# databendlabs/databend

Hardware: AMD Instinct MI355X
Metric: rows/s TPC-H Q1 hash-agg (higher is better)
Workload: dtype i64/i128 decimal

## Files before the change

### databend_amd/csrc/fagg_device.h

```cpp
#pragma once
#include "dev_expr.h"
#include "gb_device.h"

namespace {

constexpr int FA_MAX_SLOTS = 8;
constexpr int FA_KW = 4;
constexpr int FA_MAXW = 12;
constexpr int FA_MAXA = 8;
#ifndef DBHIP_JIT
constexpr int FA_ROWS = 2;
#endif

enum { W_NONE = 0, W_ADD1, W_ADD3, W_FADD, W_OR, W_MIN, W_MAX, W_CONT };
enum { C_LO = 0, C_HI, C_EXT, C_FLAG, C_ENC };

struct FaKeyTable {
  uint32_t count;
  uint32_t lock;
  uint64_t key[FA_MAX_SLOTS][FA_KW];
};
typedef volatile __attribute__((address_space(3))) FaKeyTable* FaKeyTableV;
#define FA_LDS_V(T) ((FaKeyTableV)(T))

// ... 270 lines not shown
      carry = (uint64_t)cout;
    }
  }
}
template <bool GENERAL, int NW>
__device__ __forceinline__ void fa_wave_fold(uint64_t (&v)[NW], const uint32_t (&wm)[NW]) {
#pragma nounroll
  for (int off = 32; off >= 1; off >>= 1) {
    uint64_t o[NW];
#pragma unroll
    for (int w = 0; w < NW; ++w) o[w] = __shfl_xor(v[w], off, 64);
    fa_fold_words<GENERAL, NW>(v, o, wm);
  }
}

template <int SLOTS, bool GENERAL, int NW, bool DIV = false>
__device__ __forceinline__ void fagg_body(const FaArgs& A) {
  extern __shared__ uint64_t ex_lds[];
  __shared__ FaKeyTable T;
  __shared__ uint32_t wm_lds[FA_MAXW];
  __shared__ uint32_t wg_touched;
  __shared__ unsigned long long wg_row0;
  __shared__ uint64_t fa_xw[4][SLOTS][NW];
#ifdef DBHIP_JIT
  const FaArgs& M = kM;
  uint64_t ex_rf[EX_MAX_SLOTS * FA_ROWS];
  uint64_t* const ex_regs = ex_rf;
#define EX_REG(r, k) ex_regs[(r) * FA_ROWS + (k)]
#else
  const FaArgs& M = A;
  uint64_t* const ex_regs = ex_lds;
#define EX_REG(r, k) ex_regs[((r) * FA_ROWS + (k)) * 256 + tid]
#endif
  const ExProg& P = M.P;
  const ExProg& PA = A.P;
  const int tid = threadIdx.x, lane = tid & 63;
  if (tid == 0) { T.count = 0; T.lock = 0; wg_touched = 0; }
  if (tid < FA_MAX_SLOTS * FA_KW) T.key[tid / FA_KW][tid % FA_KW] = 0;
  if (tid < FA_MAXW) wm_lds[tid] = M.wm[tid];
  __syncthreads();

  uint32_t wm[NW];
#pragma unroll
  for (int w = 0; w < NW; ++w) {
#ifdef DBHIP_JIT
    wm[w] = M.wm[w];
#else
    wm[w] = __builtin_amdgcn_readfirstlane(A.wm[w]);
#endif
  }
  uint64_t acc[SLOTS][NW];
  uint32_t touched = 0;
// ... 198 lines not shown
              }
            } else if (GENERAL && op == W_CONT && WM_COMP(m) == C_FLAG) {
            } else {
              const unsigned long long cin = WM_CARRY(m) ? (unsigned long long)carry : 0ULL;
              unsigned long long cout;
              acc[g][w] = (uint64_t)__builtin_addcll((unsigned long long)acc[g][w], (unsigned long long)val[w], cin, &cout);
              carry = (uint64_t)cout;
            }
          }
        }
      }
    }
  }
  flags = (uint32_t)fa_wave_or((uint64_t)flags);
  if (lane == 0 && flags) atomicOr((unsigned long long*)&A.ctrl[1], (unsigned long long)flags);
  const uint32_t wt = (uint32_t)fa_wave_or((uint64_t)touched);
  if (lane == 0 && wt) atomicOr(&wg_touched, wt);
  const int wave = tid >> 6;
#pragma unroll
  for (int g = 0; g < SLOTS; ++g) {
    if ((wt >> g) & 1) fa_wave_fold<GENERAL, NW>(acc[g], wm);
    if (lane == 0) {
#pragma unroll
      for (int w = 0; w < NW; ++w) fa_xw[wave][g][w] = acc[g][w];
    }
  }
  __syncthreads();
  const uint32_t tw = wg_touched;
  if (tw == 0) return;
  if (tid == 0) wg_row0 = atomicAdd((unsigned long long*)&A.ctrl[0], (unsigned long long)__popc(tw));
  __syncthreads();
  if (tid < SLOTS && ((tw >> tid) & 1)) {
    const int g = tid;
    uint64_t v[NW];
#pragma unroll
    for (int w = 0; w < NW; ++w) v[w] = fa_xw[0][g][w];
#pragma unroll
    for (int x = 1; x < 4; ++x) {
      uint64_t o[NW];
#pragma unroll
      for (int w = 0; w < NW; ++w) o[w] = fa_xw[x][g][w];
      fa_fold_words<GENERAL, NW>(v, o, wm);
    }
    uint64_t* r = A.partial_rows + (wg_row0 + (unsigned long long)__popc(tw & ((1u << g) - 1u))) * M.W;
    uint64_t kk[FA_KW];
#pragma unroll
    for (int j = 0; j < FA_KW; ++j) kk[j] = T.key[g][j];
    uint64_t vmk = ~0ULL;
#pragma unroll
    for (int j = 0; j < FA_KW; ++j)
      if (j == M.validity_word) vmk = kk[j];
    uint64_t h = 0;
    for (int q = 0; q < M.nkeys; ++q) {
      uint64_t w2[2] = {0, 0};
#pragma unroll
      for (int j = 0; j < FA_KW; ++j) {
        if (j == M.key_off[q]) w2[0] = kk[j];
        if (M.key_words[q] == 2 && j == M.key_off[q] + 1) w2[1] = kk[j];
      }
      const uint64_t hk = gb_hash_words(M.key_type[q], w2, (vmk >> q) & 1);
      h = q == 0 ? hk : merge_hash(h, hk);
    }
#pragma unroll
    for (int j = 0; j < FA_KW; ++j)
      if (j < M.nkey_words) r[j] = kk[j];
    r[M.hash_word] = h;
    uint64_t* st = r + M.state_off;
#pragma unroll
    for (int w = 0; w < NW; ++w) {
      if (w >= M.nwords) continue;
      const uint32_t op = WM_OP(wm[w]);
      if (op == W_NONE) continue;
      const bool flag = op == W_OR || (GENERAL && op == W_CONT && WM_COMP(wm[w]) == C_FLAG);
      st[w] = flag ? (v[w] ? 1 : 0) : v[w];
    }
  }
#undef EX_REG
#undef FA_IN_DATA
#undef FA_IN_VALID
#undef FA_IN_VOFF
#undef FA_KEY_DATA
#undef FA_KEY_VALID
#undef FA_KEY_VOFF
#undef FA_FILTER_BITS
#undef FA_FILTER_OFF
}

#ifndef DBHIP_JIT
template <int SLOTS, bool GENERAL, int NW, bool DIV = false>
__global__ __launch_bounds__(256, (SLOTS * NW <= 16) ? 2 : 1) void fagg_kernel(FaArgs A) {
  fagg_body<SLOTS, GENERAL, NW, DIV>(A);
}
#endif

}
```

### databend_amd/csrc/gbk_merge_lds.h

```cpp

namespace {

int32_t ensure(void** p, size_t* cap, size_t bytes) {
  if (*cap >= bytes) return DBHIP_OK;
  if (*p) {
    int32_t rc = dbhip_free(*p);
    if (rc) return rc;
    *p = nullptr; *cap = 0;
  }
  size_t want = bytes + (bytes >> 3) + 256;
  int32_t rc = dbhip_alloc(want, p);
  if (rc) { *p = nullptr; return rc; }
  *cap = want;
  return DBHIP_OK;
}

int32_t alloc_table(dbhip_groupby* g, int64_t cap, hipStream_t s) {
  uint64_t* nh = nullptr;
  uint64_t* nr = nullptr;
  int32_t rc = dbhip_alloc((size_t)cap * 8, (void**)&nh);
  if (rc == DBHIP_OK) rc = dbhip_alloc((size_t)cap * g->L.W * 8, (void**)&nr);
  hipError_t e = rc == DBHIP_OK ? hipMemsetAsync(nh, 0, (size_t)cap * 8, s) : hipSuccess;
  if (rc != DBHIP_OK || e != hipSuccess) {
    if (nh) (void)dbhip_free(nh);
// ... 140 lines not shown
  g->arena_cap = want;
  return DBHIP_OK;
}
int32_t reserve_arena_for_chunk(dbhip_groupby* g, hipStream_t s) {
  uint64_t lb = 0;
  DBHIP_CHECK(hipMemcpyAsync(&lb, &g->ctrl[9], 8, hipMemcpyDeviceToHost, s));
  DBHIP_CHECK(hipStreamSynchronize(s));
  if (lb == 0) return DBHIP_OK;
  g->has_long = 1;
  return reserve_arena(g, lb, s);
}
bool layout_has_strings(const GbLayout& L) { return L.str_w1_mask != 0; }
bool layout_has_wide_minmax(const GbLayout& L);

int32_t merge_rows_unpinned(dbhip_groupby* g, const uint64_t* rows_in, int64_t n, hipStream_t s, const uint64_t* n_dev, const uint64_t* abort_dev,
                            int deferred = 0);
int32_t merge_rows(dbhip_groupby* g, const uint64_t* rows_in, int64_t n, hipStream_t s,
                   const uint64_t* n_dev = nullptr, const uint64_t* abort_dev = nullptr) {
  int32_t rc = merge_rows_unpinned(g, rows_in, n, s, n_dev, abort_dev);
  if (rc == DBHIP_OK && n > 0) rc = pin_string_states(g, s);
  return rc;
}
int32_t merge_rows_unpinned(dbhip_groupby* g, const uint64_t* rows_in, int64_t n, hipStream_t s,
                            const uint64_t* n_dev, const uint64_t* abort_dev, int deferred) {
  if (n == 0) return DBHIP_OK;
  if (n > 0xFFFFFFF0LL) {
    set_error("groupby: more than 2^32 rows in one call");
    return DBHIP_ERR_INVALID;
  }
  int32_t rc;
  if ((rc = ensure((void**)&g->gid, &g->gid_cap, (size_t)n * 4))) return rc;
  if ((rc = ensure((void**)&g->retry, &g->retry_cap, (size_t)n * 4))) return rc;
  const int grid = grid_for(n, 256);
  uint64_t* host_ctrl = pinned_words(0);
  if (!host_ctrl) return DBHIP_ERR_HIP;
  const uint64_t* cur_rows = rows_in;
  int64_t cur_n = n;
  const DevCount dc{n_dev, abort_dev};
  if ((deferred || (g->count_host + n) * 135 <= g->cap * 100) && n <= 256) {
    hipLaunchKernelGGL(gb_merge_small_kernel, dim3(1), dim3(256), 0, s, g->L, cur_rows, cur_n, g->slot_hash, g->rows, g->cap, g->hash_mask, g->gid,
                       g->retry, g->ctrl, dc, g->arena);
    DBHIP_LAUNCH_CHECK();
    if (deferred) return DBHIP_OK;
    DBHIP_CHECK(hipMemcpyAsync(host_ctrl, g->ctrl, 5 * sizeof(uint64_t), hipMemcpyDeviceToHost, s));
    DBHIP_CHECK(hipStreamSynchronize(s));
    g->count_host = (int64_t)host_ctrl[0];
    if (host_ctrl[3] & 2) {
      set_error("groupby: a string key longer than 12 bytes was met; keep the CPU operator for this block");
      return DBHIP_ERR_UNSUPPORTED;
    }
    if (host_ctrl[1]) {
      set_error("groupby: collision chain filled the table during retry; create the table with a larger capacity");
      return DBHIP_ERR_CAPACITY;
    }
    return DBHIP_OK;
  }
  if (deferred || (g->count_host + n) * 135 <= g->cap * 100) {
    DBHIP_CHECK(hipMemsetAsync(&g->ctrl[1], 0, 16, s));
    hipLaunchKernelGGL(gb_probe_kernel, dim3(grid), dim3(256), 0, s, g->L, cur_rows, cur_n, g->slot_hash, g->rows, g->cap,
                       g->hash_mask, g->gid, g->ctrl, dc, g->arena);
    if (deferred == 1 || (!deferred && g->count_host > 0 && g->count_host <= 32 && n <= 65536) || n <= 2048 || layout_has_wide_minmax(g->L))
      hipLaunchKernelGGL(gb_accum_lowcard_kernel, dim3(deferred == 1 && grid > 16 ? 16 : grid), dim3(256), 0, s, g->L, cur_rows, cur_n, g->rows, g->gid, g->retry,
                         g->ctrl, dc, g->arena);
    else
      hipLaunchKernelGGL(gb_accum_kernel, dim3(grid), dim3(256), 0, s, g->L, cur_rows, cur_n, g->rows, g->gid, g->retry, g->ctrl, dc, g->arena);
    hipLaunchKernelGGL(gb_retry_kernel, dim3(1), dim3(64), 0, s, g->L, cur_rows, g->slot_hash, g->rows, g->cap, g->hash_mask,
                       g->gid, g->retry, g->ctrl, g->arena);
    DBHIP_LAUNCH_CHECK();
    if (deferred) return DBHIP_OK;
    DBHIP_CHECK(hipMemcpyAsync(host_ctrl, g->ctrl, 5 * sizeof(uint64_t), hipMemcpyDeviceToHost, s));
// ... 315 lines not shown
```

### databend_amd/csrc/gbk_rows.h

```cpp

namespace {

struct HashCols {
  GbCol c[GB_MAX_KEYS];
  int n;
};

__global__ __launch_bounds__(256) void group_hash_kernel(HashCols hc, int64_t n, uint64_t* out,
                                                         unsigned long long* bad) {
  constexpr int U = 4;
  const int64_t T = (int64_t)gridDim.x * blockDim.x;
  const int64_t t = (int64_t)blockIdx.x * blockDim.x + threadIdx.x;
  for (int64_t base = 0; base < n; base += U * T) {
    int64_t row[U];
    bool in[U];
    uint64_t h[U];
#pragma unroll
    for (int u = 0; u < U; ++u) {
      row[u] = base + u * T + t;
      in[u] = row[u] < n;
      if (!in[u]) row[u] = n - 1;
      h[u] = 0;
    }
    for (int k = 0; k < hc.n; ++k) {
// ... 452 lines not shown
      }
      pos = (pos + 1) & cmask;
    }
    if (!done) ctrl[1] |= 2;
  }
}
__global__ void gb_retry_kernel(GbLayout L, const uint64_t* rows_in, uint64_t* slot_hash, uint64_t* rows,
                                int64_t cap, uint64_t hash_mask, const uint32_t* gid,
                                const uint32_t* retry, uint64_t* ctrl, uint8_t* arena) {
  if (threadIdx.x != 0 || blockIdx.x != 0) return;
  gb_retry_body(L, rows_in, slot_hash, rows, cap, hash_mask, gid, retry, ctrl, arena);
}

__global__ __launch_bounds__(256) void gb_merge_small_kernel(GbLayout L, const uint64_t* rows_in, int64_t n, uint64_t* slot_hash, uint64_t* rows,
                                                             int64_t cap, uint64_t hash_mask, uint32_t* gid, uint32_t* retry, uint64_t* ctrl,
                                                             DevCount dc, uint8_t* arena) {
  n = dev_rows(dc, n);
  if (threadIdx.x < 2) ctrl[1 + threadIdx.x] = 0;
  __threadfence();
  __syncthreads();
  gb_probe_body(L, rows_in, n, slot_hash, rows, cap, hash_mask, gid, ctrl, arena);
  __threadfence();
  __syncthreads();
  gb_accum_lowcard_body(L, rows_in, n, rows, gid, retry, ctrl, arena);
  __threadfence();
  __syncthreads();
  if (threadIdx.x == 0) gb_retry_body(L, rows_in, slot_hash, rows, cap, hash_mask, gid, retry, ctrl, arena);
}

__global__ __launch_bounds__(256) void gb_rehash_kernel(GbLayout L, const uint64_t* old_hash,
                                                        const uint64_t* old_rows, int64_t old_cap,
                                                        uint64_t* new_hash, uint64_t* new_rows,
                                                        int64_t new_cap, uint64_t hash_mask) {
  const uint64_t cmask = (uint64_t)new_cap - 1;
  for (int64_t s = (int64_t)blockIdx.x * blockDim.x + threadIdx.x; s < old_cap;
       s += (int64_t)gridDim.x * blockDim.x) {
    uint64_t hw = old_hash[s];
    if (hw == 0) continue;
    const uint64_t* r = old_rows + s * L.W;
    uint64_t pos = home_slot(probe_word(r[L.hash_word], hash_mask), new_cap);
    while (true) {
      unsigned long long old = atomicCAS((unsigned long long*)&new_hash[pos], 0ULL, (unsigned long long)hw);
// ... 501 lines not shown
```

### databend_amd/csrc/k_fagg.hip

```cpp
#include "fagg_device.h"
#include "runtime.h"

#include <dirent.h>
#include <dlfcn.h>
#include <errno.h>
#include <sys/stat.h>
#include <fcntl.h>
#include <signal.h>
#include <spawn.h>
#include <sys/wait.h>
#include <unistd.h>

#include <atomic>
#include <chrono>
#include <deque>
#include <map>
#include <mutex>
#include <string>

#include <stdlib.h>
#include <string.h>
#include <time.h>

using namespace dbhip;

int32_t dbhip_groupby_merge_rows_dev_internal(dbhip_groupby* g, const uint64_t* rows, int64_t n_max, const uint64_t* n_dev,
                                              const uint64_t* abort_dev, hipStream_t s);
int32_t dbhip_groupby_merge_rows_internal(dbhip_groupby* g, const uint64_t* rows, int64_t n, hipStream_t s);
int64_t dbhip_groupby_capacity_internal(dbhip_groupby* g);
int32_t dbhip_groupby_reserve_merge_internal(dbhip_groupby* g, int64_t n);
int64_t dbhip_groupby_count_internal(dbhip_groupby* g);
const GbLayout* dbhip_groupby_layout_internal(dbhip_groupby* g);
int32_t dbhip_groupby_merge_rows_deferred_internal(dbhip_groupby* g, const uint64_t* rows, int64_t n_max, const uint64_t* n_dev,
                                                   const uint64_t* abort_dev, hipStream_t s);
int32_t dbhip_groupby_ensure_room_internal(dbhip_groupby* g, int64_t extra, hipStream_t s);
uint64_t* dbhip_groupby_ctrl_internal(dbhip_groupby* g);
void dbhip_groupby_set_count_internal(dbhip_groupby* g, int64_t count);
void** dbhip_groupby_pipe_slot_internal(dbhip_groupby* g);

namespace {

#include "build/jit_embed.inc"

struct JitOut {
  std::string s;
  void num(long long v) { s += std::to_string(v); s += ","; }
  void u64(uint64_t v) { char b[40]; snprintf(b, sizeof(b), "0x%llxULL,", (unsigned long long)v); s += b; }
  void null() { s += "nullptr,"; }
  void open() { s += "{"; }
  void close() { s += "},"; }
};

void jit_ins(JitOut& o, const ExIns& I) {
// ... 271 lines not shown
  return ok;
}

struct JitEntry {
  enum State { ABSENT = 0, PENDING, READY, FAILED } state = ABSENT;
  hipModule_t mod = nullptr;
  hipFunction_t fn = nullptr;
  std::chrono::steady_clock::time_point checked{}, started{};
};
std::mutex g_jit_mu;
std::map<std::string, JitEntry> g_jit_cache;

int jit_mode() {
  static const int m = [] {
    const char* e = getenv("DBHIP_FAGG_JIT");
    if (!e) return 1;
    if (!strcmp(e, "sync")) return 2;
    return atoi(e) == 0 ? 0 : 1;
  }();
  return m;
}

enum { JIT_LOOKUP = 0, JIT_COMPILE = 1, JIT_BACKGROUND = 2 };
void fa_shape(const FaArgs& A, FaArgs& K) {
  K = A;
  for (int i = 0; i < EX_MAX_INPUTS; ++i) { K.P.in_data[i] = nullptr; K.P.in_valid[i] = nullptr; K.P.in_voff[i] = 0; }
  K.P.err_words = nullptr; K.P.err_count = nullptr;
  for (int k = 0; k < FA_KW; ++k) { K.key[k].data = nullptr; K.key[k].validity = nullptr; K.key[k].voff = 0; K.key[k].buffers = nullptr; }
  K.filter_bits = nullptr; K.filter_off = 0; K.n = 0; K.partial_rows = nullptr; K.ctrl = nullptr; K.blocks = nullptr; K.wgs_per_block = 0;
}
hipFunction_t jit_kernel(const FaArgs& A, int slots, bool general, int nw, int how, bool* pending = nullptr, bool multi = false) {
  if (pending) *pending = false;
  const int mode = jit_mode();
  if (mode == 0) return nullptr;
  if (mode == 2) how = JIT_COMPILE;
// ... 78 lines not shown
  return words <= FA_MAXW && L.hash_word == L.nkey_words && L.agg_off[0] == L.hash_word + 1;
}

static std::atomic<uint64_t> g_fa_jit_launches{0}, g_fa_interp_launches{0}, g_fa_pending_refusals{0}, g_fa_multi_blocks{0};
extern "C" int32_t dbhip_fagg_stats(uint64_t* out3_host) {
  DBHIP_REQUIRE(out3_host, "dbhip_fagg_stats: NULL argument");
  out3_host[0] = g_fa_jit_launches.load(); out3_host[1] = g_fa_interp_launches.load(); out3_host[2] = g_fa_pending_refusals.load();
  return DBHIP_OK;
}

static thread_local bool t_prepare_only = false;
static thread_local bool t_jit_only = false;
static thread_local bool t_jit_pending = false;
static thread_local bool t_jit_may_compile = true;

static int32_t fa_build_args(const GbLayout& L, const dbhip_col* keys, const dbhip_agg_program* prog, FaArgs& A, bool* out_general,
                             int* out_nwords, bool* out_may_raise) {
  ExRoot roots[EX_MAX_ROOTS + 1];
  int n_roots = 0, filter_root = -1;
  int root_of_agg[FA_MAXA];
  if (prog->filter_reg >= 0) { roots[n_roots].reg = prog->filter_reg; filter_root = n_roots++; }
  for (int a = 0; a < L.naggs; ++a) {
    root_of_agg[a] = -1;
    const int32_t r = prog->arg_regs[a];
    if (r == DBHIP_ARG_NONE) {
      if (L.agg_kind[a] != DBHIP_AGG_COUNT) { set_error("dbhip_groupby_add_block_program: aggregate %d needs an argument", a); return DBHIP_ERR_INVALID; }
      continue;
    }
    if (n_roots >= EX_MAX_ROOTS) { set_error("dbhip_groupby_add_block_program: more than %d program results", EX_MAX_ROOTS); return DBHIP_ERR_UNSUPPORTED; }
    roots[n_roots].reg = r;
// ... 1 lines not shown
  }
  bool may_raise = false, any_nullable = false;
  if (n_roots == 0) {
    set_error("dbhip_groupby_add_block_program: nothing to evaluate (count(*) only): use dbhip_groupby_add_block_filtered");
    return DBHIP_ERR_UNSUPPORTED;
  }
  int32_t rc = dbhip_expr_compile_internal(prog->prog, prog->n_ins, prog->inputs, prog->n_inputs, roots, n_roots, filter_root, &A.P,
                                           &may_raise, &any_nullable);
  if (rc) return rc;
  A.naggs = L.naggs;
  int nwords = 0;
  bool general = false;
  for (int a = 0; a < L.naggs; ++a) {
    int slot = 0, wide = 0, sgn = 0, enc_type = L.agg_type[a];
    uint32_t dep = 0;
    const int fw = L.agg_flag[a];
    const int base_words = L.agg_words[a] - (fw ? 1 : 0);
    if (root_of_agg[a] >= 0) {
      const ExRoot& R = roots[root_of_agg[a]];
      if (L.agg_kind[a] != DBHIP_AGG_COUNT) {
        if (R.type != L.agg_type[a] || !fa_arg_type_ok(R.type)) {
          set_error("dbhip_groupby_add_block_program: aggregate %d expects an argument of type %d, the program yields type %d", a, L.agg_type[a], R.type);
          return DBHIP_ERR_INVALID;
        }
      }
      slot = R.slot; wide = R.wide; dep = R.dep;
      sgn = R.type == DBHIP_T_DEC128 || type_class(R.type) == CLS_SIGNED;
      if (R.type == DBHIP_T_F32) enc_type = DBHIP_T_F64;
    }
    auto put = [&](int op, int comp, int carry_in) {
      A.wm[nwords++] = (uint32_t)op | ((uint32_t)comp << 3) | ((uint32_t)slot << 6) | ((uint32_t)wide << 12) | ((uint32_t)sgn << 13) |
                       ((uint32_t)carry_in << 14) | (1u << 15) | ((dep & 255u) << 16) | (((uint32_t)enc_type & 31u) << 24);
    };
    switch (L.agg_kind[a]) {
      case DBHIP_AGG_COUNT: put(W_ADD1, C_FLAG, 0); break;
      case DBHIP_AGG_SUM:
        if (base_words == 3) { put(W_ADD3, C_LO, 0); put(W_CONT, C_HI, 1); put(W_CONT, C_EXT, 1); }
        else if (L.agg_type[a] == DBHIP_T_F32 || L.agg_type[a] == DBHIP_T_F64) { put(W_FADD, C_LO, 0); general = true; }
        else put(W_ADD1, C_LO, 0);
        if (fw) put(W_OR, C_FLAG, 0);
        break;
      case DBHIP_AGG_MIN: case DBHIP_AGG_MAX:
        if (L.agg_words[a] >= 3) { set_error("fused aggregation: min / max over Decimal128 / Decimal256 / String stays on the row path"); return DBHIP_ERR_UNSUPPORTED; }
        if (L.agg_kind[a] == DBHIP_AGG_MIN) put(W_MIN, C_ENC, 0); else put(W_MAX, C_ENC, 0);
        put(W_CONT, C_FLAG, 0); general = true; break;
    }
  }
  A.nwords = nwords;
  A.state_off = L.agg_off[0];
  A.nkeys = L.nkeys; A.nkey_words = L.nkey_words; A.validity_word = L.validity_word; A.hash_word = L.hash_word; A.W = L.W;
  for (int k = 0; k < L.nkeys; ++k) {
    if (keys[k].type != L.key_type[k]) { set_error("dbhip_groupby_add_block_program: key %d has type %d, table expects %d", k, keys[k].type, L.key_type[k]); return DBHIP_ERR_INVALID; }
    if (keys[k].validity && !L.key_nullable[k]) { set_error("dbhip_groupby_add_block_program: key %d carries validity but was declared NOT NULL", k); return DBHIP_ERR_INVALID; }
    GbCol& c = A.key[k];
    c.data = keys[k].data; c.validity = keys[k].validity; c.voff = keys[k].validity_offset; c.buffers = keys[k].buffers;
    c.type = keys[k].type; c.is_scalar = keys[k].is_scalar;
    A.key_type[k] = L.key_type[k]; A.key_off[k] = L.key_off[k]; A.key_words[k] = L.key_words[k];
    A.key_has_valid[k] = keys[k].validity != nullptr;
  }
  *out_general = general; *out_nwords = nwords; *out_may_raise = may_raise;
  return DBHIP_OK;
// ... 20 lines not shown
#define FA_LAUNCH(SL, GEN)                                                                                     \
  do {                                                                                                         \
    if (nwords <= 4) hipLaunchKernelGGL((fagg_kernel<SL, GEN, 4>), dim3(grid), dim3(256), lds, s, A);           \
    else hipLaunchKernelGGL((fagg_kernel<SL, GEN, FA_MAXW>), dim3(grid), dim3(256), lds, s, A);                 \
  } while (0)
  bool has_div = false;
  for (int i = 0; i < A.P.n_ins; ++i) has_div |= A.P.ins[i].op == EX_DEC && dec_op_needs_division(A.P.dec[A.P.ins[i].dec_idx]);
  if (has_div && slots == 4) hipLaunchKernelGGL((fagg_kernel<4, true, FA_MAXW, true>), dim3(grid), dim3(256), lds, s, A);
  else if (has_div) hipLaunchKernelGGL((fagg_kernel<8, true, FA_MAXW, true>), dim3(grid), dim3(256), lds, s, A);
  else if (slots == 4 && !general) FA_LAUNCH(4, false);
  else if (slots == 4) FA_LAUNCH(4, true);
  else if (!general) FA_LAUNCH(8, false);
  else FA_LAUNCH(8, true);
#undef FA_LAUNCH
  return DBHIP_OK;
}

namespace {
constexpr int FA_PIPE_WINDOW = 2048;
constexpr int FA_PIPE_BATCH = 512;
constexpr size_t FA_PIPE_COPY_BYTES = 16384;
constexpr size_t FA_PIPE_TABLE_BYTES = 65536;
constexpr int FA_PIPE_RING = 8;
constexpr int64_t FA_PIPE_BIG = 8 << 20;
constexpr int64_t FA_PIPE_BATCH_ROWS = 32 << 20;
struct FaShape { FaArgs A; bool general; int nwords; size_t lds; std::string sig; };
struct FaPending { int shape; FaBlock b; };
struct FaMerge { uint64_t seq; int64_t rows_ub; int64_t blocks; };
struct FaPipe {
  bool on = false, bound = false, slots8 = false;
// ... 358 lines not shown
  int32_t rc = fa_build_args(L, keys, prog, A, &general, &nwords, &may_raise);
  if (rc) return rc;
  A.filter_bits = filter_bitmap; A.filter_off = filter_bit_offset; A.n = n;
  A.has_filter = filter_bitmap != nullptr;
  const size_t lds = (size_t)(A.P.n_slots > 6 ? A.P.n_slots : 6) * FA_ROWS * 256 * 8;
  if (lds > 60 * 1024) {
    set_error("dbhip_groupby_add_block_program: %d live LDS slots exceed the register file; split the expression", A.P.n_slots);
    return DBHIP_ERR_UNSUPPORTED;
  }
  const int64_t nchunks = ceil_div(n, 64 * FA_ROWS);
  const int grid = (int)(ceil_div(nchunks, 4) < 512 ? ceil_div(nchunks, 4) : 512);
  if (FaPipe* pp = (FaPipe*)*dbhip_groupby_pipe_slot_internal(g); pp && !t_prepare_only) {
    int64_t committed = 0;
    if ((rc = fa_pipe_checkpoint(g, pp, &committed, true))) return rc;
  }
  const size_t rows_bytes = (size_t)grid * FA_MAX_SLOTS * L.W * 8;
  uint8_t* ws = (uint8_t*)scratch(rows_bytes + 64, 6, s);
  if (!ws) return DBHIP_ERR_HIP;
  uint64_t* ctrl = (uint64_t*)ws;
  A.ctrl = ctrl;
  A.partial_rows = (uint64_t*)(ws + 64);
  A.P.err_words = nullptr;
  A.P.err_count = (unsigned long long*)&ctrl[2];
  uint64_t* host_ctrl = pinned_words(1);
  if (!host_ctrl) return DBHIP_ERR_HIP;
  host_ctrl[0] = host_ctrl[1] = host_ctrl[2] = 0;
  const int64_t n_max = (int64_t)grid * FA_MAX_SLOTS;
  const bool chained = (dbhip_groupby_count_internal(g) + n_max) * 135 <= dbhip_groupby_capacity_internal(g) * 100;
  if ((rc = dbhip_groupby_reserve_merge_internal(g, n_max))) return rc;
  if (t_prepare_only) {
    (void)jit_kernel(A, dbhip_groupby_count_internal(g) > 4 ? 8 : 4, general, nwords, JIT_COMPILE);
    if (FaPipe* pq = (FaPipe*)*dbhip_groupby_pipe_slot_internal(g); pq && pq->on)
      (void)jit_kernel(A, dbhip_groupby_count_internal(g) > 4 ? 8 : 4, general, nwords, JIT_COMPILE, nullptr, true);
    return DBHIP_OK;
  }
  for (int variant = dbhip_groupby_count_internal(g) > 4 ? 1 : 0; variant < 2; ++variant) {
    DBHIP_CHECK(hipMemsetAsync(ctrl, 0, 64, s));
    kernel_timer_start(s);
    if ((rc = fa_launch(A, variant == 0 ? 4 : 8, general, nwords, grid, lds, s))) return rc;
    kernel_timer_stop(s);
    DBHIP_LAUNCH_CHECK();
    DBHIP_CHECK(hipMemcpyAsync(host_ctrl, ctrl, 24, hipMemcpyDeviceToHost, s));
    if (chained && !may_raise) {
      rc = dbhip_groupby_merge_rows_dev_internal(g, A.partial_rows, n_max, &ctrl[0], &ctrl[1], s);
      if (rc) return rc;
      if (!(host_ctrl[1] & 3)) return DBHIP_OK;
    } else {
      DBHIP_CHECK(hipStreamSynchronize(s));
    }
    if (!(host_ctrl[1] & 1)) break;
  }
  if (host_ctrl[1] & 2) {
    set_error("dbhip_groupby_add_block_program: a group key string is longer than 12 bytes");
    return DBHIP_ERR_UNSUPPORTED;
  }
  if (host_ctrl[1] & 1) {
    set_error("dbhip_groupby_add_block_program: more than %d distinct groups inside one workgroup; use the operator-at-a-time path", FA_MAX_SLOTS);
    return DBHIP_ERR_CAPACITY;
  }
  if (host_ctrl[2]) {
    set_error("dbhip_groupby_add_block_program: %llu row error(s) in the fused maps (Decimal overflow / divided by zero); "
              "evaluate the maps with dbhip_expr_eval to get the rows", (unsigned long long)host_ctrl[2]);
// ... 211 lines not shown
```

### databend_amd/csrc/k_groupby.hip

```cpp
#include <mutex>
#include "gb_device.h"
#include "runtime.h"

#include <math.h>
#include <stdlib.h>
#include <string.h>

#include <new>
#include <vector>

using namespace dbhip;

#define GB_INVALID_SLOT 0xFFFFFFFFu

struct dbhip_groupby {
  int64_t hint_groups;
  GbLayout L;
  int64_t cap;
  uint64_t* slot_hash;
  uint64_t* rows;
  uint64_t* ctrl;
  uint64_t hash_mask;
  int64_t count_host;
  uint64_t* rows_in; size_t rows_in_cap;
// ... 59 lines not shown
  return merge_rows(g, rows, n, s);
}
int32_t dbhip_groupby_merge_rows_dev_internal(dbhip_groupby* g, const uint64_t* rows, int64_t n_max, const uint64_t* n_dev,
                                              const uint64_t* abort_dev, hipStream_t s) {
  return merge_rows(g, rows, n_max, s, n_dev, abort_dev);
}
int32_t dbhip_groupby_reserve_merge_internal(dbhip_groupby* g, int64_t n) {
  int32_t rc;
  if ((rc = ensure((void**)&g->gid, &g->gid_cap, (size_t)n * 4))) return rc;
  return ensure((void**)&g->retry, &g->retry_cap, (size_t)n * 4);
}
int32_t dbhip_groupby_merge_rows_deferred_internal(dbhip_groupby* g, const uint64_t* rows, int64_t n_max, const uint64_t* n_dev,
                                                   const uint64_t* abort_dev, hipStream_t s) {
  return merge_rows_unpinned(g, rows, n_max, s, n_dev, abort_dev, 1);
}
int32_t dbhip_groupby_ensure_room_internal(dbhip_groupby* g, int64_t extra, hipStream_t s) {
  uint64_t cnt = 0;
  DBHIP_CHECK(hipMemcpyAsync(&cnt, &g->ctrl[0], 8, hipMemcpyDeviceToHost, s));
  DBHIP_CHECK(hipStreamSynchronize(s));
  g->count_host = (int64_t)cnt;
  while ((g->count_host + extra) * 135 > g->cap * 100) {
    const int32_t rc = grow(g, s);
    if (rc) return rc;
  }
  return DBHIP_OK;
}
uint64_t* dbhip_groupby_ctrl_internal(dbhip_groupby* g) { return g->ctrl; }
void dbhip_groupby_set_count_internal(dbhip_groupby* g, int64_t count) { g->count_host = count; }
void** dbhip_groupby_pipe_slot_internal(dbhip_groupby* g) { return &g->fa_pipe; }
int64_t dbhip_groupby_capacity_internal(dbhip_groupby* g) { return g->cap; }
// ... 5 lines not shown
```

### databend_amd/csrc/k_q1.hip

```cpp
#include "gb_device.h"
#include "runtime.h"

#include <stdlib.h>
#include <string.h>

using namespace dbhip;

int32_t dbhip_groupby_merge_rows_internal(dbhip_groupby* g, const uint64_t* rows, int64_t n, hipStream_t s);
int32_t dbhip_groupby_merge_rows_dev_internal(dbhip_groupby* g, const uint64_t* rows, int64_t n_max, const uint64_t* n_dev,
                                              const uint64_t* abort_dev, hipStream_t s);
int64_t dbhip_groupby_capacity_internal(dbhip_groupby* g);
int64_t dbhip_groupby_count_internal(dbhip_groupby* g);
const GbLayout* dbhip_groupby_layout_internal(dbhip_groupby* g);

namespace {

constexpr int MAX_SLOTS = 8;
constexpr int Q1_W = 15;

struct alignas(16) U4 {
  uint32_t x, y, z, w;
};
struct alignas(16) L2 {
  int64_t a, b;
};
struct alignas(8) I2 {
  int32_t a, b;
};
// ... 289 lines not shown
  bool layout_ok = L->nkeys == 2 && L->naggs == 6 && L->W == Q1_W && L->key_type[0] == DBHIP_T_STRING &&
                   L->key_type[1] == DBHIP_T_STRING && L->agg_off[0] == 5 && L->agg_off[2] == 7 &&
                   L->agg_off[5] == 14 && L->agg_words[2] == 3 && L->agg_words[3] == 3;
  DBHIP_REQUIRE(layout_ok, "dbhip_q1_fused: table was not created by dbhip_q1_create_groupby");
  if (n == 0) return DBHIP_OK;
  DBHIP_REQUIRE(l_quantity && l_extendedprice && l_discount && l_tax && l_returnflag_views &&
                    l_linestatus_views && l_shipdate,
                "dbhip_q1_fused: NULL column");
  uintptr_t al = (uintptr_t)l_quantity | (uintptr_t)l_extendedprice | (uintptr_t)l_discount |
                 (uintptr_t)l_tax | (uintptr_t)l_returnflag_views | (uintptr_t)l_linestatus_views;
  DBHIP_REQUIRE((al & 15) == 0 && ((uintptr_t)l_shipdate & 7) == 0,
                "dbhip_q1_fused: columns must be 16-byte aligned (shipdate 8-byte)");
  hipStream_t s = resolve_stream(stream);
  const int64_t ntiles = ceil_div(n, 128);
  const int grid = (int)(ceil_div(ntiles, 4) < 512 ? ceil_div(ntiles, 4) : 512);
  size_t rows_bytes = (size_t)grid * MAX_SLOTS * Q1_W * 8;
  uint8_t* ws = (uint8_t*)scratch(rows_bytes + 64, 4, s);
  if (!ws) return DBHIP_ERR_HIP;
  uint64_t* ctrl = (uint64_t*)ws;
  uint64_t* partial = (uint64_t*)(ws + 64);
  Q1Args A;
  A.qty = l_quantity; A.price = l_extendedprice; A.disc = l_discount; A.tax = l_tax;
  A.rf = (const U4*)l_returnflag_views; A.ls = (const U4*)l_linestatus_views;
  A.shipdate = l_shipdate; A.cutoff = shipdate_cutoff; A.n = n;
  A.partial_rows = partial; A.ctrl = ctrl;
  uint64_t* host_ctrl = pinned_words(1);
  if (!host_ctrl) return DBHIP_ERR_HIP;
  host_ctrl[0] = host_ctrl[1] = 0;
  const int64_t n_max4 = (int64_t)grid * 4, n_max8 = (int64_t)grid * MAX_SLOTS;
  const bool chained = (dbhip_groupby_count_internal(g) + n_max8) * 135 <= dbhip_groupby_capacity_internal(g) * 100;
  for (int variant = 0; variant < 2; ++variant) {
    DBHIP_CHECK(hipMemsetAsync(ctrl, 0, 64, s));
    kernel_timer_start(s);
    if (variant == 0) hipLaunchKernelGGL(q1_fused_kernel, dim3(grid), dim3(256), 0, s, A);
    else hipLaunchKernelGGL(q1_fused_kernel_8slots, dim3(grid), dim3(256), 0, s, A);
    kernel_timer_stop(s);
    DBHIP_LAUNCH_CHECK();
    DBHIP_CHECK(hipMemcpyAsync(host_ctrl, ctrl, 16, hipMemcpyDeviceToHost, s));
    if (chained) {
      int32_t rc = dbhip_groupby_merge_rows_dev_internal(g, partial, variant == 0 ? n_max4 : n_max8, &ctrl[0], &ctrl[1], s);
      if (rc) return rc;
      if (!(host_ctrl[1] & 3)) return DBHIP_OK;
    } else {
      DBHIP_CHECK(hipStreamSynchronize(s));
    }
    if (!(host_ctrl[1] & 1)) break;
  }
  if (host_ctrl[1] & 2) {
    set_error("dbhip_q1_fused: a group key string is longer than 12 bytes; use the operator-at-a-time path");
    return DBHIP_ERR_UNSUPPORTED;
  }
  if (host_ctrl[1] & 1) {
    set_error("dbhip_q1_fused: more than %d distinct groups inside one workgroup; use the operator-at-a-time path", MAX_SLOTS);
    return DBHIP_ERR_CAPACITY;
  }
  return dbhip_groupby_merge_rows_internal(g, partial, (int64_t)host_ctrl[0], s);
}

// ... 2 lines not shown
```

Baseline: 94.11 billion.

## Fold per-workgroup partial rows on device before merging into group table

Adds a single-workgroup kernel that folds all per-workgroup partial rows into at most eight group rows. The small merge kernel then copies its control words into a report buffer, so one host sync reads everything. Previously up to grid×slots partial rows went through the general merge path, and host control was read separately. The change adds an extra kernel launch and a serial fold over all partial rows in one workgroup, with a fallback when the fold overflows slots.

```diff
diff --git a/databend_amd/csrc/fagg_device.h b/databend_amd/csrc/fagg_device.h
--- a/databend_amd/csrc/fagg_device.h
+++ b/databend_amd/csrc/fagg_device.h
@@ -308,14 +308,57 @@
   }
 }
 
+template <int SLOTS, bool GENERAL, int NW>
+__device__ __forceinline__ uint32_t fa_wg_fold(uint64_t (&acc)[SLOTS][NW], uint32_t touched, const uint32_t (&wm)[NW], uint64_t (&v)[NW]) {
+  __shared__ uint32_t wg_touched;
+  __shared__ uint64_t fa_xw[4][SLOTS][NW];
+  const int tid = threadIdx.x, lane = tid & 63, wave = tid >> 6;
+  if (tid == 0) wg_touched = 0;
+  __syncthreads();
+  const uint32_t wt = (uint32_t)fa_wave_or((uint64_t)touched);
+  if (lane == 0 && wt) atomicOr(&wg_touched, wt);
+#pragma unroll
+  for (int g = 0; g < SLOTS; ++g) {
+    if ((wt >> g) & 1) fa_wave_fold<GENERAL, NW>(acc[g], wm);
+    if (lane == 0) {
+#pragma unroll
+      for (int w = 0; w < NW; ++w) fa_xw[wave][g][w] = acc[g][w];
+    }
+  }
+  __syncthreads();
+  const uint32_t tw = wg_touched;
+  if (tid < SLOTS && ((tw >> tid) & 1)) {
+    const int g = tid;
+#pragma unroll
+    for (int w = 0; w < NW; ++w) v[w] = fa_xw[0][g][w];
+#pragma unroll
+    for (int x = 1; x < 4; ++x) {
+      uint64_t o[NW];
+#pragma unroll
+      for (int w = 0; w < NW; ++w) o[w] = fa_xw[x][g][w];
+      fa_fold_words<GENERAL, NW>(v, o, wm);
+    }
+  }
+  return tw;
+}
+template <bool GENERAL, int NW>
+__device__ __forceinline__ void fa_write_state(uint64_t* st, const uint64_t (&v)[NW], const uint32_t (&wm)[NW], int nwords) {
+#pragma unroll
+  for (int w = 0; w < NW; ++w) {
+    if (w >= nwords) continue;
+    const uint32_t op = WM_OP(wm[w]);
+    if (op == W_NONE) continue;
+    const bool flag = op == W_OR || (GENERAL && op == W_CONT && WM_COMP(wm[w]) == C_FLAG);
+    st[w] = flag ? (v[w] ? 1 : 0) : v[w];
+  }
+}
+
 template <int SLOTS, bool GENERAL, int NW, bool DIV = false>
 __device__ __forceinline__ void fagg_body(const FaArgs& A) {
   extern __shared__ uint64_t ex_lds[];
   __shared__ FaKeyTable T;
   __shared__ uint32_t wm_lds[FA_MAXW];
-  __shared__ uint32_t wg_touched;
   __shared__ unsigned long long wg_row0;
-  __shared__ uint64_t fa_xw[4][SLOTS][NW];
 #ifdef DBHIP_JIT
   const FaArgs& M = kM;
   uint64_t ex_rf[EX_MAX_SLOTS * FA_ROWS];
@@ -329,7 +372,7 @@
   const ExProg& P = M.P;
   const ExProg& PA = A.P;
   const int tid = threadIdx.x, lane = tid & 63;
-  if (tid == 0) { T.count = 0; T.lock = 0; wg_touched = 0; }
+  if (tid == 0) { T.count = 0; T.lock = 0; }
   if (tid < FA_MAX_SLOTS * FA_KW) T.key[tid / FA_KW][tid % FA_KW] = 0;
   if (tid < FA_MAXW) wm_lds[tid] = M.wm[tid];
   __syncthreads();
@@ -558,34 +601,13 @@
   }
   flags = (uint32_t)fa_wave_or((uint64_t)flags);
   if (lane == 0 && flags) atomicOr((unsigned long long*)&A.ctrl[1], (unsigned long long)flags);
-  const uint32_t wt = (uint32_t)fa_wave_or((uint64_t)touched);
-  if (lane == 0 && wt) atomicOr(&wg_touched, wt);
-  const int wave = tid >> 6;
-#pragma unroll
-  for (int g = 0; g < SLOTS; ++g) {
-    if ((wt >> g) & 1) fa_wave_fold<GENERAL, NW>(acc[g], wm);
-    if (lane == 0) {
-#pragma unroll
-      for (int w = 0; w < NW; ++w) fa_xw[wave][g][w] = acc[g][w];
-    }
-  }
-  __syncthreads();
-  const uint32_t tw = wg_touched;
+  uint64_t v[NW];
+  const uint32_t tw = fa_wg_fold<SLOTS, GENERAL, NW>(acc, touched, wm, v);
   if (tw == 0) return;
   if (tid == 0) wg_row0 = atomicAdd((unsigned long long*)&A.ctrl[0], (unsigned long long)__popc(tw));
   __syncthreads();
   if (tid < SLOTS && ((tw >> tid) & 1)) {
     const int g = tid;
-    uint64_t v[NW];
-#pragma unroll
-    for (int w = 0; w < NW; ++w) v[w] = fa_xw[0][g][w];
-#pragma unroll
-    for (int x = 1; x < 4; ++x) {
-      uint64_t o[NW];
-#pragma unroll
-      for (int w = 0; w < NW; ++w) o[w] = fa_xw[x][g][w];
-      fa_fold_words<GENERAL, NW>(v, o, wm);
-    }
     uint64_t* r = A.partial_rows + (wg_row0 + (unsigned long long)__popc(tw & ((1u << g) - 1u))) * M.W;
     uint64_t kk[FA_KW];
 #pragma unroll
@@ -609,15 +631,7 @@
     for (int j = 0; j < FA_KW; ++j)
       if (j < M.nkey_words) r[j] = kk[j];
     r[M.hash_word] = h;
-    uint64_t* st = r + M.state_off;
-#pragma unroll
-    for (int w = 0; w < NW; ++w) {
-      if (w >= M.nwords) continue;
-      const uint32_t op = WM_OP(wm[w]);
-      if (op == W_NONE) continue;
-      const bool flag = op == W_OR || (GENERAL && op == W_CONT && WM_COMP(wm[w]) == C_FLAG);
-      st[w] = flag ? (v[w] ? 1 : 0) : v[w];
-    }
+    fa_write_state<GENERAL, NW>(r + M.state_off, v, wm, M.nwords);
   }
 #undef EX_REG
 #undef FA_IN_DATA
@@ -635,6 +649,76 @@
 __global__ __launch_bounds__(256, (SLOTS * NW <= 16) ? 2 : 1) void fagg_kernel(FaArgs A) {
   fagg_body<SLOTS, GENERAL, NW, DIV>(A);
 }
+
+constexpr int FA_CTRL_WORDS = 16;
+struct FaFoldArgs {
+  int32_t W, nkey_words, hash_word, state_off, nwords;
+  uint32_t wm[FA_MAXW];
+};
+template <int NW>
+__global__ __launch_bounds__(256) void fa_fold_partials_kernel(FaFoldArgs F, const uint64_t* rows, uint64_t* ctrl, uint64_t* out) {
+  __shared__ FaKeyTable T;
+  __shared__ uint64_t hash_of[FA_MAX_SLOTS];
+  __shared__ uint32_t wg_flags;
+  const int tid = threadIdx.x;
+  if (tid == 0) { T.count = 0; T.lock = 0; wg_flags = 0; }
+  if (tid < FA_MAX_SLOTS * FA_KW) T.key[tid / FA_KW][tid % FA_KW] = 0;
+  __syncthreads();
+  const uint64_t n = ctrl[0];
+  if (ctrl[1] & 3) return;
+  uint32_t wm[NW];
+#pragma unroll
+  for (int w = 0; w < NW; ++w) wm[w] = __builtin_amdgcn_readfirstlane(w < F.nwords ? F.wm[w] : 0u);
+  uint64_t acc[FA_MAX_SLOTS][NW];
+#pragma unroll
+  for (int g = 0; g < FA_MAX_SLOTS; ++g)
+#pragma unroll
+    for (int w = 0; w < NW; ++w) acc[g][w] = 0;
+  uint32_t touched = 0, flags = 0;
+  FaCache<FA_MAX_SLOTS> C;
+  C.refresh(&T);
+  for (uint64_t r0 = 0; r0 < n; r0 += 256) {
+    const uint64_t i = r0 + (uint64_t)tid;
+    const bool want[1] = {i < n};
+    const uint64_t* r = rows + (want[0] ? i : 0) * (uint64_t)F.W;
+    uint64_t kw[1][FA_KW];
+#pragma unroll
+    for (int j = 0; j < FA_KW; ++j) kw[0][j] = (want[0] && j < F.nkey_words) ? r[j] : 0;
+    if (__builtin_amdgcn_readfirstlane(FA_LDS_V(&T)->count) != C.nk) C.refresh(&T);
+    int slot[1];
+    fa_resolve_all<FA_MAX_SLOTS, 1>(&T, C, want, kw, slot, flags);
+    if (__ballot((flags & 1u) != 0)) break;
+    uint64_t val[NW];
+#pragma unroll
+    for (int w = 0; w < NW; ++w) val[w] = (want[0] && w < F.nwords) ? r[F.state_off + w] : 0;
+#pragma unroll
+    for (int g = 0; g < FA_MAX_SLOTS; ++g) {
+      if (slot[0] == g) {
+        touched |= 1u << g;
+        hash_of[g] = r[F.hash_word];
+        fa_fold_words<false, NW>(acc[g], val, wm);
+      }
+    }
+  }
+  flags = (uint32_t)fa_wave_or((uint64_t)flags);
+  if ((tid & 63) == 0 && flags) atomicOr(&wg_flags, flags);
+  uint64_t v[NW];
+  const uint32_t tw = fa_wg_fold<FA_MAX_SLOTS, false, NW>(acc, touched, wm, v);
+  if (wg_flags & 1u) {
+    if (tid == 0) ctrl[5] = 1;
+    return;
+  }
+  if (tid == 0) ctrl[4] = (uint64_t)__popc(tw);
+  if (tid < FA_MAX_SLOTS && ((tw >> tid) & 1)) {
+    const int g = tid;
+    uint64_t* d = out + (uint64_t)__popc(tw & ((1u << g) - 1u)) * (uint64_t)F.W;
+#pragma unroll
+    for (int j = 0; j < FA_KW; ++j)
+      if (j < F.nkey_words) d[j] = T.key[g][j];
+    d[F.hash_word] = hash_of[g];
+    fa_write_state<false, NW>(d + F.state_off, v, wm, F.nwords);
+  }
+}
 #endif
 
 }
diff --git a/databend_amd/csrc/gbk_merge_lds.h b/databend_amd/csrc/gbk_merge_lds.h
--- a/databend_amd/csrc/gbk_merge_lds.h
+++ b/databend_amd/csrc/gbk_merge_lds.h
@@ -178,15 +178,27 @@
 bool layout_has_wide_minmax(const GbLayout& L);
 
 int32_t merge_rows_unpinned(dbhip_groupby* g, const uint64_t* rows_in, int64_t n, hipStream_t s, const uint64_t* n_dev, const uint64_t* abort_dev,
-                            int deferred = 0);
+                            int deferred = 0, uint64_t* report_dev = nullptr);
 int32_t merge_rows(dbhip_groupby* g, const uint64_t* rows_in, int64_t n, hipStream_t s,
                    const uint64_t* n_dev = nullptr, const uint64_t* abort_dev = nullptr) {
   int32_t rc = merge_rows_unpinned(g, rows_in, n, s, n_dev, abort_dev);
   if (rc == DBHIP_OK && n > 0) rc = pin_string_states(g, s);
   return rc;
 }
+int32_t merge_report(dbhip_groupby* g, const uint64_t* host_ctrl) {
+  g->count_host = (int64_t)host_ctrl[0];
+  if (host_ctrl[3] & 2) {
+    set_error("groupby: a string key longer than 12 bytes was met; keep the CPU operator for this block");
+    return DBHIP_ERR_UNSUPPORTED;
+  }
+  if (host_ctrl[1]) {
+    set_error("groupby: collision chain filled the table during retry; create the table with a larger capacity");
+    return DBHIP_ERR_CAPACITY;
+  }
+  return DBHIP_OK;
+}
 int32_t merge_rows_unpinned(dbhip_groupby* g, const uint64_t* rows_in, int64_t n, hipStream_t s,
-                            const uint64_t* n_dev, const uint64_t* abort_dev, int deferred) {
+                            const uint64_t* n_dev, const uint64_t* abort_dev, int deferred, uint64_t* report_dev) {
   if (n == 0) return DBHIP_OK;
   if (n > 0xFFFFFFF0LL) {
     set_error("groupby: more than 2^32 rows in one call");
@@ -203,21 +215,16 @@
   const DevCount dc{n_dev, abort_dev};
   if ((deferred || (g->count_host + n) * 135 <= g->cap * 100) && n <= 256) {
     hipLaunchKernelGGL(gb_merge_small_kernel, dim3(1), dim3(256), 0, s, g->L, cur_rows, cur_n, g->slot_hash, g->rows, g->cap, g->hash_mask, g->gid,
-                       g->retry, g->ctrl, dc, g->arena);
+                       g->retry, g->ctrl, dc, g->arena, report_dev);
     DBHIP_LAUNCH_CHECK();
     if (deferred) return DBHIP_OK;
     DBHIP_CHECK(hipMemcpyAsync(host_ctrl, g->ctrl, 5 * sizeof(uint64_t), hipMemcpyDeviceToHost, s));
     DBHIP_CHECK(hipStreamSynchronize(s));
-    g->count_host = (int64_t)host_ctrl[0];
-    if (host_ctrl[3] & 2) {
-      set_error("groupby: a string key longer than 12 bytes was met; keep the CPU operator for this block");
-      return DBHIP_ERR_UNSUPPORTED;
-    }
-    if (host_ctrl[1]) {
-      set_error("groupby: collision chain filled the table during retry; create the table with a larger capacity");
-      return DBHIP_ERR_CAPACITY;
-    }
-    return DBHIP_OK;
+    return merge_report(g, host_ctrl);
+  }
+  if (report_dev) {
+    set_error("groupby: a reported merge takes at most 256 rows");
+    return DBHIP_ERR_INVALID;
   }
   if (deferred || (g->count_host + n) * 135 <= g->cap * 100) {
     DBHIP_CHECK(hipMemsetAsync(&g->ctrl[1], 0, 16, s));
diff --git a/databend_amd/csrc/gbk_rows.h b/databend_amd/csrc/gbk_rows.h
--- a/databend_amd/csrc/gbk_rows.h
+++ b/databend_amd/csrc/gbk_rows.h
@@ -490,7 +490,7 @@
 
 __global__ __launch_bounds__(256) void gb_merge_small_kernel(GbLayout L, const uint64_t* rows_in, int64_t n, uint64_t* slot_hash, uint64_t* rows,
                                                              int64_t cap, uint64_t hash_mask, uint32_t* gid, uint32_t* retry, uint64_t* ctrl,
-                                                             DevCount dc, uint8_t* arena) {
+                                                             DevCount dc, uint8_t* arena, uint64_t* report) {
   n = dev_rows(dc, n);
   if (threadIdx.x < 2) ctrl[1 + threadIdx.x] = 0;
   __threadfence();
@@ -502,6 +502,10 @@
   __threadfence();
   __syncthreads();
   if (threadIdx.x == 0) gb_retry_body(L, rows_in, slot_hash, rows, cap, hash_mask, gid, retry, ctrl, arena);
+  if (threadIdx.x == 0 && report) {
+    __threadfence();
+    for (int i = 0; i < 5; ++i) report[i] = __hip_atomic_load(&ctrl[i], __ATOMIC_RELAXED, __HIP_MEMORY_SCOPE_AGENT);
+  }
 }
 
 __global__ __launch_bounds__(256) void gb_rehash_kernel(GbLayout L, const uint64_t* old_hash,
diff --git a/databend_amd/csrc/k_fagg.hip b/databend_amd/csrc/k_fagg.hip
--- a/databend_amd/csrc/k_fagg.hip
+++ b/databend_amd/csrc/k_fagg.hip
@@ -37,6 +37,9 @@
 uint64_t* dbhip_groupby_ctrl_internal(dbhip_groupby* g);
 void dbhip_groupby_set_count_internal(dbhip_groupby* g, int64_t count);
 void** dbhip_groupby_pipe_slot_internal(dbhip_groupby* g);
+int32_t dbhip_groupby_merge_rows_reported_internal(dbhip_groupby* g, const uint64_t* rows, int64_t n_max, const uint64_t* n_dev,
+                                                   const uint64_t* abort_dev, uint64_t* report_dev, hipStream_t s);
+int32_t dbhip_groupby_merge_report_internal(dbhip_groupby* g, const uint64_t* report_host);
 
 namespace {
 
@@ -338,11 +341,15 @@
 int jit_mode() {
   static const int m = [] {
     const char* e = getenv("DBHIP_FAGG_JIT");
-    if (!e) return 1;
-    if (!strcmp(e, "sync")) return 2;
+    if (!e || !strncmp(e, "nofold", 6)) return 1;
+    if (!strncmp(e, "sync", 4)) return 2;
     return atoi(e) == 0 ? 0 : 1;
   }();
   return m;
+}
+bool fa_fold_on() {
+  const char* e = getenv("DBHIP_FAGG_JIT");
+  return !(e && strstr(e, "nofold"));
 }
 
 enum { JIT_LOOKUP = 0, JIT_COMPILE = 1, JIT_BACKGROUND = 2 };
@@ -451,6 +458,43 @@
 static thread_local bool t_jit_pending = false;
 static thread_local bool t_jit_may_compile = true;
 
+static int fa_agg_words(const GbLayout& L, int a, uint32_t (&out)[4], bool* general) {
+  int n = 0;
+  auto put = [&](int op, int comp, int carry_in) { out[n++] = (uint32_t)op | ((uint32_t)comp << 3) | ((uint32_t)carry_in << 14) | (1u << 15); };
+  const int fw = L.agg_flag[a];
+  const int base_words = L.agg_words[a] - (fw ? 1 : 0);
+  switch (L.agg_kind[a]) {
+    case DBHIP_AGG_COUNT: put(W_ADD1, C_FLAG, 0); break;
+    case DBHIP_AGG_SUM:
+      if (base_words == 3) { put(W_ADD3, C_LO, 0); put(W_CONT, C_HI, 1); put(W_CONT, C_EXT, 1); }
+      else if (L.agg_type[a] == DBHIP_T_F32 || L.agg_type[a] == DBHIP_T_F64) { put(W_FADD, C_LO, 0); *general = true; }
+      else put(W_ADD1, C_LO, 0);
+      if (fw) put(W_OR, C_FLAG, 0);
+      break;
+    case DBHIP_AGG_MIN: case DBHIP_AGG_MAX:
+      if (L.agg_words[a] >= 3) return -1;
+      if (L.agg_kind[a] == DBHIP_AGG_MIN) put(W_MIN, C_ENC, 0); else put(W_MAX, C_ENC, 0);
+      put(W_CONT, C_FLAG, 0); *general = true; break;
+    default: return -1;
+  }
+  return n;
+}
+static bool fa_fold_args(const GbLayout& L, FaFoldArgs* F) {
+  if (!dbhip_fagg_layout_ok_internal(L)) return false;
+  memset(F, 0, sizeof(*F));
+  bool general = false;
+  int nwords = 0;
+  for (int a = 0; a < L.naggs; ++a) {
+    uint32_t w[4];
+    const int nw = fa_agg_words(L, a, w, &general);
+    if (nw < 0 || nwords + nw > FA_MAXW) return false;
+    for (int i = 0; i < nw; ++i) F->wm[nwords++] = w[i];
+  }
+  if (general) return false;
+  F->W = L.W; F->nkey_words = L.nkey_words; F->hash_word = L.hash_word; F->state_off = L.agg_off[0]; F->nwords = nwords;
+  return true;
+}
+
 static int32_t fa_build_args(const GbLayout& L, const dbhip_col* keys, const dbhip_agg_program* prog, FaArgs& A, bool* out_general,
                              int* out_nwords, bool* out_may_raise) {
   ExRoot roots[EX_MAX_ROOTS + 1];
@@ -482,8 +526,6 @@
   for (int a = 0; a < L.naggs; ++a) {
     int slot = 0, wide = 0, sgn = 0, enc_type = L.agg_type[a];
     uint32_t dep = 0;
-    const int fw = L.agg_flag[a];
-    const int base_words = L.agg_words[a] - (fw ? 1 : 0);
     if (root_of_agg[a] >= 0) {
       const ExRoot& R = roots[root_of_agg[a]];
       if (L.agg_kind[a] != DBHIP_AGG_COUNT) {
@@ -496,23 +538,14 @@
       sgn = R.type == DBHIP_T_DEC128 || type_class(R.type) == CLS_SIGNED;
       if (R.type == DBHIP_T_F32) enc_type = DBHIP_T_F64;
     }
-    auto put = [&](int op, int comp, int carry_in) {
-      A.wm[nwords++] = (uint32_t)op | ((uint32_t)comp << 3) | ((uint32_t)slot << 6) | ((uint32_t)wide << 12) | ((uint32_t)sgn << 13) |
-                       ((uint32_t)carry_in << 14) | (1u << 15) | ((dep & 255u) << 16) | (((uint32_t)enc_type & 31u) << 24);
-    };
-    switch (L.agg_kind[a]) {
-      case DBHIP_AGG_COUNT: put(W_ADD1, C_FLAG, 0); break;
-      case DBHIP_AGG_SUM:
-        if (base_words == 3) { put(W_ADD3, C_LO, 0); put(W_CONT, C_HI, 1); put(W_CONT, C_EXT, 1); }
-        else if (L.agg_type[a] == DBHIP_T_F32 || L.agg_type[a] == DBHIP_T_F64) { put(W_FADD, C_LO, 0); general = true; }
-        else put(W_ADD1, C_LO, 0);
-        if (fw) put(W_OR, C_FLAG, 0);
-        break;
-      case DBHIP_AGG_MIN: case DBHIP_AGG_MAX:
-        if (L.agg_words[a] >= 3) { set_error("fused aggregation: min / max over Decimal128 / Decimal256 / String stays on the row path"); return DBHIP_ERR_UNSUPPORTED; }
-        if (L.agg_kind[a] == DBHIP_AGG_MIN) put(W_MIN, C_ENC, 0); else put(W_MAX, C_ENC, 0);
-        put(W_CONT, C_FLAG, 0); general = true; break;
-    }
+    uint32_t base[4];
+    bool gen = false;
+    const int nw = fa_agg_words(L, a, base, &gen);
+    if (nw < 0) { set_error("fused aggregation: min / max over Decimal128 / Decimal256 / String stays on the row path"); return DBHIP_ERR_UNSUPPORTED; }
+    general |= gen;
+    for (int i = 0; i < nw; ++i)
+      A.wm[nwords++] = base[i] | ((uint32_t)slot << 6) | ((uint32_t)wide << 12) | ((uint32_t)sgn << 13) | ((dep & 255u) << 16) |
+                       (((uint32_t)enc_type & 31u) << 24);
   }
   A.nwords = nwords;
   A.state_off = L.agg_off[0];
@@ -563,6 +596,19 @@
   else FA_LAUNCH(8, true);
 #undef FA_LAUNCH
   return DBHIP_OK;
+}
+
+int32_t dbhip_fagg_fold_queue_internal(dbhip_groupby* g, const uint64_t* partial, uint64_t* ctrl, uint64_t* folded, hipStream_t s) {
+  FaFoldArgs F;
+  if (!fa_fold_on() || !fa_fold_args(*dbhip_groupby_layout_internal(g), &F)) return -1;
+  if (F.nwords <= 4) hipLaunchKernelGGL((fa_fold_partials_kernel<4>), dim3(1), dim3(256), 0, s, F, partial, ctrl, folded);
+  else hipLaunchKernelGGL((fa_fold_partials_kernel<FA_MAXW>), dim3(1), dim3(256), 0, s, F, partial, ctrl, folded);
+  DBHIP_LAUNCH_CHECK();
+  return dbhip_groupby_merge_rows_reported_internal(g, folded, FA_MAX_SLOTS, &ctrl[4], &ctrl[1], &ctrl[8], s);
+}
+int32_t dbhip_fagg_fold_finish_internal(dbhip_groupby* g, const uint64_t* partial, const uint64_t* host_ctrl, hipStream_t s) {
+  if (host_ctrl[5]) return dbhip_groupby_merge_rows_internal(g, partial, (int64_t)host_ctrl[0], s);
+  return dbhip_groupby_merge_report_internal(g, host_ctrl + 8);
 }
 
 namespace {
@@ -951,12 +997,13 @@
     int64_t committed = 0;
     if ((rc = fa_pipe_checkpoint(g, pp, &committed, true))) return rc;
   }
-  const size_t rows_bytes = (size_t)grid * FA_MAX_SLOTS * L.W * 8;
-  uint8_t* ws = (uint8_t*)scratch(rows_bytes + 64, 6, s);
+  const size_t rows_bytes = (size_t)grid * FA_MAX_SLOTS * L.W * 8, folded_bytes = (size_t)FA_MAX_SLOTS * L.W * 8;
+  uint8_t* ws = (uint8_t*)scratch(FA_CTRL_WORDS * 8 + folded_bytes + rows_bytes, 6, s);
   if (!ws) return DBHIP_ERR_HIP;
   uint64_t* ctrl = (uint64_t*)ws;
+  uint64_t* folded = (uint64_t*)(ws + FA_CTRL_WORDS * 8);
   A.ctrl = ctrl;
-  A.partial_rows = (uint64_t*)(ws + 64);
+  A.partial_rows = (uint64_t*)(ws + FA_CTRL_WORDS * 8 + folded_bytes);
   A.P.err_words = nullptr;
   A.P.err_count = (unsigned long long*)&ctrl[2];
   uint64_t* host_ctrl = pinned_words(1);
@@ -977,12 +1024,21 @@
     if ((rc = fa_launch(A, variant == 0 ? 4 : 8, general, nwords, grid, lds, s))) return rc;
     kernel_timer_stop(s);
     DBHIP_LAUNCH_CHECK();
-    DBHIP_CHECK(hipMemcpyAsync(host_ctrl, ctrl, 24, hipMemcpyDeviceToHost, s));
     if (chained && !may_raise) {
-      rc = dbhip_groupby_merge_rows_dev_internal(g, A.partial_rows, n_max, &ctrl[0], &ctrl[1], s);
-      if (rc) return rc;
-      if (!(host_ctrl[1] & 3)) return DBHIP_OK;
+      rc = general ? -1 : dbhip_fagg_fold_queue_internal(g, A.partial_rows, ctrl, folded, s);
+      if (rc > 0) return rc;
+      if (rc == 0) {
+        DBHIP_CHECK(hipMemcpyAsync(host_ctrl, ctrl, FA_CTRL_WORDS * 8, hipMemcpyDeviceToHost, s));
+        DBHIP_CHECK(hipStreamSynchronize(s));
+        if (!(host_ctrl[1] & 3)) return dbhip_fagg_fold_finish_internal(g, A.partial_rows, host_ctrl, s);
+      } else {
+        DBHIP_CHECK(hipMemcpyAsync(host_ctrl, ctrl, 24, hipMemcpyDeviceToHost, s));
+        rc = dbhip_groupby_merge_rows_dev_internal(g, A.partial_rows, variant == 0 ? (int64_t)grid * 4 : n_max, &ctrl[0], &ctrl[1], s);
+        if (rc) return rc;
+        if (!(host_ctrl[1] & 3)) return DBHIP_OK;
+      }
     } else {
+      DBHIP_CHECK(hipMemcpyAsync(host_ctrl, ctrl, 24, hipMemcpyDeviceToHost, s));
       DBHIP_CHECK(hipStreamSynchronize(s));
     }
     if (!(host_ctrl[1] & 1)) break;
diff --git a/databend_amd/csrc/k_groupby.hip b/databend_amd/csrc/k_groupby.hip
--- a/databend_amd/csrc/k_groupby.hip
+++ b/databend_amd/csrc/k_groupby.hip
@@ -97,6 +97,11 @@
                                                    const uint64_t* abort_dev, hipStream_t s) {
   return merge_rows_unpinned(g, rows, n_max, s, n_dev, abort_dev, 1);
 }
+int32_t dbhip_groupby_merge_rows_reported_internal(dbhip_groupby* g, const uint64_t* rows, int64_t n_max, const uint64_t* n_dev,
+                                                   const uint64_t* abort_dev, uint64_t* report_dev, hipStream_t s) {
+  return merge_rows_unpinned(g, rows, n_max, s, n_dev, abort_dev, 1, report_dev);
+}
+int32_t dbhip_groupby_merge_report_internal(dbhip_groupby* g, const uint64_t* report_host) { return merge_report(g, report_host); }
 int32_t dbhip_groupby_ensure_room_internal(dbhip_groupby* g, int64_t extra, hipStream_t s) {
   uint64_t cnt = 0;
   DBHIP_CHECK(hipMemcpyAsync(&cnt, &g->ctrl[0], 8, hipMemcpyDeviceToHost, s));
diff --git a/databend_amd/csrc/k_q1.hip b/databend_amd/csrc/k_q1.hip
--- a/databend_amd/csrc/k_q1.hip
+++ b/databend_amd/csrc/k_q1.hip
@@ -12,6 +12,8 @@
 int64_t dbhip_groupby_capacity_internal(dbhip_groupby* g);
 int64_t dbhip_groupby_count_internal(dbhip_groupby* g);
 const GbLayout* dbhip_groupby_layout_internal(dbhip_groupby* g);
+int32_t dbhip_fagg_fold_queue_internal(dbhip_groupby* g, const uint64_t* partial, uint64_t* ctrl, uint64_t* folded, hipStream_t s);
+int32_t dbhip_fagg_fold_finish_internal(dbhip_groupby* g, const uint64_t* partial, const uint64_t* host_ctrl, hipStream_t s);
 
 namespace {
 
@@ -331,11 +333,12 @@
   hipStream_t s = resolve_stream(stream);
   const int64_t ntiles = ceil_div(n, 128);
   const int grid = (int)(ceil_div(ntiles, 4) < 512 ? ceil_div(ntiles, 4) : 512);
-  size_t rows_bytes = (size_t)grid * MAX_SLOTS * Q1_W * 8;
-  uint8_t* ws = (uint8_t*)scratch(rows_bytes + 64, 4, s);
+  size_t rows_bytes = (size_t)grid * MAX_SLOTS * Q1_W * 8, folded_bytes = (size_t)MAX_SLOTS * Q1_W * 8;
+  uint8_t* ws = (uint8_t*)scratch(128 + folded_bytes + rows_bytes, 4, s);
   if (!ws) return DBHIP_ERR_HIP;
   uint64_t* ctrl = (uint64_t*)ws;
-  uint64_t* partial = (uint64_t*)(ws + 64);
+  uint64_t* folded = (uint64_t*)(ws + 128);
+  uint64_t* partial = (uint64_t*)(ws + 128 + folded_bytes);
   Q1Args A;
   A.qty = l_quantity; A.price = l_extendedprice; A.disc = l_discount; A.tax = l_tax;
   A.rf = (const U4*)l_returnflag_views; A.ls = (const U4*)l_linestatus_views;
@@ -353,12 +356,21 @@
     else hipLaunchKernelGGL(q1_fused_kernel_8slots, dim3(grid), dim3(256), 0, s, A);
     kernel_timer_stop(s);
     DBHIP_LAUNCH_CHECK();
-    DBHIP_CHECK(hipMemcpyAsync(host_ctrl, ctrl, 16, hipMemcpyDeviceToHost, s));
     if (chained) {
-      int32_t rc = dbhip_groupby_merge_rows_dev_internal(g, partial, variant == 0 ? n_max4 : n_max8, &ctrl[0], &ctrl[1], s);
-      if (rc) return rc;
-      if (!(host_ctrl[1] & 3)) return DBHIP_OK;
+      int32_t rc = dbhip_fagg_fold_queue_internal(g, partial, ctrl, folded, s);
+      if (rc > 0) return rc;
+      if (rc == 0) {
+        DBHIP_CHECK(hipMemcpyAsync(host_ctrl, ctrl, 128, hipMemcpyDeviceToHost, s));
+        DBHIP_CHECK(hipStreamSynchronize(s));
+        if (!(host_ctrl[1] & 3)) return dbhip_fagg_fold_finish_internal(g, partial, host_ctrl, s);
+      } else {
+        DBHIP_CHECK(hipMemcpyAsync(host_ctrl, ctrl, 16, hipMemcpyDeviceToHost, s));
+        rc = dbhip_groupby_merge_rows_dev_internal(g, partial, variant == 0 ? n_max4 : n_max8, &ctrl[0], &ctrl[1], s);
+        if (rc) return rc;
+        if (!(host_ctrl[1] & 3)) return DBHIP_OK;
+      }
     } else {
+      DBHIP_CHECK(hipMemcpyAsync(host_ctrl, ctrl, 16, hipMemcpyDeviceToHost, s));
       DBHIP_CHECK(hipStreamSynchronize(s));
     }
     if (!(host_ctrl[1] & 1)) break;
```

Result: no change. 93.69 billion (-0.4%).
